# Daniel-Liu-c0deb0t/cute-nucleotides

Hardware: AMD Instinct MI355X
Metric: Gnt/s encode+decode on 16 GiB random ACGT; % HBM read roofline at 1/8 GPU (higher is better)
Workload: dtype u8

## Files before the change

### hip/counted_output.hpp

```cpp
#pragma once

#include <hip/hip_runtime.h>
#include <stdint.h>

#include <algorithm>
#include <initializer_list>

#include "util_kernels.hpp"
#include "word_tile.hpp"

namespace cnt {

constexpr int kCountedScanBlock = 1024, kCountedGroup = 16;

__device__ __forceinline__ uint64_t counted_tile_base(const uint64_t* offs, const uint32_t* counts, uint64_t tile) {
    uint64_t b = offs[tile / kCountedGroup];
    const uint32_t* g = counts + (tile - tile % kCountedGroup);
#pragma unroll
    for (int q = 0; q < kCountedGroup - 1; ++q) b += (uint64_t)q < tile % kCountedGroup ? g[q] : 0u;
    return b;
}

__global__ __launch_bounds__(kCountedScanBlock) void counted_scan(const uint32_t* __restrict__ counts, uint64_t* __restrict__ offs,
                                                                  uint64_t n_tiles, uint64_t* __restrict__ count) {
    __shared__ uint64_t s_w[kCountedScanBlock / 64];
    const uint32_t lane = threadIdx.x & 63, wave = threadIdx.x >> 6;
    const uint64_t n_groups = (n_tiles + kCountedGroup - 1) / kCountedGroup;
    uint64_t carry = 0;
    for (uint64_t first = 0; first < n_groups; first += kCountedScanBlock) {
        const uint64_t g = first + threadIdx.x;
        uint64_t sum = 0;
        if (g < n_groups) {
            const u32x4* q = reinterpret_cast<const u32x4*>(counts + g * kCountedGroup);
#pragma unroll
            for (int u = 0; u < kCountedGroup / 4; ++u) {
                const u32x4 c = q[u];
#pragma unroll
                for (int e = 0; e < 4; ++e) sum += g * kCountedGroup + 4 * u + e < n_tiles ? c[e] : 0u;
            }
        }
        uint64_t x = sum;
#pragma unroll
        for (int o = 1; o < 64; o <<= 1) {
            const uint64_t y = shfl_up_u64(x, o);
            if (lane >= (uint32_t)o) x += y;
        }
        if (lane == 63) s_w[wave] = x;
        __syncthreads();
        uint64_t before = carry + x - sum, total = 0;
#pragma unroll
        for (int q = 0; q < kCountedScanBlock / 64; ++q) {
            const uint64_t y = s_w[q];
            before += q < (int)wave ? y : 0;
            total += y;
        }
        if (g < n_groups) offs[g] = before;
        carry += total;
        __syncthreads();
    }
    if (threadIdx.x == 0) *count = carry;
}

inline uint64_t counted_scratch_bytes(uint64_t n_tiles) {
    if (!n_tiles) return 0;
    const uint64_t groups = (n_tiles + kCountedGroup - 1) / kCountedGroup;
    return 16 + ((groups + 1) & ~1ull) * 8 + groups * kCountedGroup * 4;
}

struct CountedScratch {
    uint64_t* offs;
    uint32_t* counts;
    void* behind;
};
inline CountedScratch counted_carve(void* d_work, uint64_t n_tiles) {
    const uint64_t groups = (n_tiles + kCountedGroup - 1) / kCountedGroup;
    uint64_t* offs = reinterpret_cast<uint64_t*>((reinterpret_cast<uintptr_t>(d_work) + 15) & ~(uintptr_t)15);
    uint32_t* counts = reinterpret_cast<uint32_t*>(offs + ((groups + 1) & ~1ull));
    return {offs, counts, counts + groups * kCountedGroup};
}

inline void counted_scan_enqueue(const CountedScratch& w, uint64_t n_tiles, void* d_count, hipStream_t s) {
    hipLaunchKernelGGL(counted_scan, dim3(1), dim3(kCountedScanBlock), 0, s, w.counts, w.offs, n_tiles, static_cast<uint64_t*>(d_count));
}

struct CountedOut {
    const void* p;
    bool required;
};
inline int counted_args(const void* bits, size_t len, std::initializer_list<CountedOut> outs, uint64_t most, size_t out_cap, const void* count) {
    if (!bits || !count || !aligned(bits, 8) || !aligned(count, 8)) return CNT_EINVAL;
    for (const CountedOut& o : outs)
        if ((o.required && !o.p) || !aligned(o.p, 8)) return CNT_EINVAL;
    const size_t in_bytes = cnt_words_for(len) * 8, out_bytes = std::min<uint64_t>(most, out_cap) * 8;
    if (overlaps(count, 8, bits, in_bytes)) return CNT_EINVAL;
    for (const CountedOut* o = outs.begin(); o != outs.end(); ++o) {
        if (!o->p) continue;
        if (overlaps(bits, in_bytes, o->p, out_bytes) || overlaps(count, 8, o->p, out_bytes)) return CNT_EINVAL;
        for (const CountedOut* e = outs.begin(); e != o; ++e)
            if (e->p && overlaps(e->p, out_bytes, o->p, out_bytes)) return CNT_EINVAL;
    }
    return CNT_OK;
}

inline int counted_work(const void* d_work, size_t work_bytes, size_t need, const void* bits, size_t len, std::initializer_list<const void*> outs,
                        uint64_t most, size_t out_cap, const void* count) {
    if (work_bytes < need || !d_work) return CNT_EINVAL;
    if (overlaps(d_work, need, bits, cnt_words_for(len) * 8) || overlaps(d_work, need, count, 8)) return CNT_EINVAL;
    for (const void* o : outs)
        if (o && overlaps(d_work, need, o, std::min<uint64_t>(most, out_cap) * 8)) return CNT_EINVAL;
    return CNT_OK;
}
// ... 23 lines not shown
```

### hip/orf_kernels.hpp

```cpp
#pragma once

#include <hip/hip_runtime.h>
#include <stdint.h>

#include "codec2_kernels.hpp"
#include "counted_output.hpp"
#include "find_kernels.hpp"

namespace cnt {

constexpr int kOrfBlock = 256;
constexpr int kOrfWaves = kOrfBlock / 64;
constexpr uint64_t kOrfTileWords = kOrfBlock, kOrfTile = 32 * kOrfTileWords;
constexpr int kOrfCarryBlock = 1024;
constexpr int kOrfPairs = 6;
constexpr uint32_t kOrfOpenEnd = 0x400u, kOrfNoStop = 0x800u;
constexpr uint64_t kOrfNone = ~0ull;
static_assert(kOrfTile + 1 < (1u << 16), "a position of a tile, plus one, is half a dword");

struct OrfArgs {
    const uint8_t* in;
    uint64_t words, len;
    uint64_t stops[2], starts[2];
    uint64_t min_len;
    uint64_t n_tiles;
    uint32_t* sums;
    uint64_t* carry;
    uint32_t* counts;
    uint64_t* offs;
    uint64_t *pos, *length, *info;
    uint64_t out_cap;
};

__device__ __forceinline__ uint32_t orf_combine(uint32_t a, uint32_t b, bool rev) {
    const uint32_t sa = a & 0xFFFFu, sb = b & 0xFFFFu;
    const uint32_t st = rev ? (sb ? sb : sa) : (sa ? sa : sb);
    return (b >> 16) ? b : ((a & 0xFFFF0000u) | st);
}

struct OrfLane {
    uint64_t i0;
    uint32_t stops[2], starts[2];
    uint32_t m3;
};

__device__ __forceinline__ OrfLane orf_lane(const OrfArgs& a, uint64_t tile, uint32_t* s_tab) {
    const uint32_t j = threadIdx.x;
    if (j < 64) {
        s_tab[j] = (uint32_t)((a.stops[0] >> j) & 1u) | ((uint32_t)((a.starts[0] >> j) & 1u) << 8) | ((uint32_t)((a.stops[1] >> j) & 1u) << 16) |
                   ((uint32_t)((a.starts[1] >> j) & 1u) << 24);
    }
    const uint64_t w0 = tile * kOrfTileWords;
    uint64_t lo, hi;
    word_tile_pair<kOrfTileWords>(a.in, a.words, w0, j, lo, hi);
    __syncthreads();
    const uint32_t d[3] = {(uint32_t)lo, (uint32_t)(lo >> 32), (uint32_t)hi};
    uint32_t acc[4];
#pragma unroll
    for (int g = 0; g < 4; ++g) {
        acc[g] = 0;
#pragma unroll
        for (int r = 8 * g + 7; r >= 8 * g; --r)
            acc[g] = (acc[g] << 1) | s_tab[window_dword(d, r) & 63u];
    }
    OrfLane L;
    L.i0 = (w0 + j) * 32;
    L.m3 = (2u * (uint32_t)(tile % 3) + 2u * j) % 3u;
// ... 14 lines not shown
    const uint32_t rel = threadIdx.x * 32u + 1u, lane = threadIdx.x & 63u;
#pragma unroll
    for (int p = 0; p < kOrfPairs; ++p) {
        const int s = p / 3;
        const uint32_t mask = 0x49249249u << ((p % 3 + 3u - L.m3) % 3u);
        const uint32_t st = L.stops[s] & mask;
        const uint32_t top = st ? 31u - (uint32_t)__builtin_clz(st) : 0u;
        const uint32_t sa = L.starts[s] & mask & (st ? ~((2u << top) - 1u) : ~0u);
        const uint32_t at = s ? 31u - (uint32_t)__builtin_clz(sa | 1u) : (uint32_t)__builtin_ctz(sa | 0x80000000u);
        x[p] = (st ? (rel + top) << 16 : 0u) | (sa ? rel + at : 0u);
    }
#pragma unroll
    for (int o = 1; o < 64; o <<= 1) {
#pragma unroll
        for (int p = 0; p < kOrfPairs; ++p) {
            if (p >= 3 && !both) continue;
            const uint32_t y = __shfl_up(x[p], o, 64);
            if (lane >= (uint32_t)o) x[p] = orf_combine(y, x[p], p >= 3);
        }
    }
}

__global__ __launch_bounds__(kOrfBlock) void orf_summary(OrfArgs a, uint64_t first_tile) {
    __shared__ uint32_t s_tab[64];
    __shared__ uint32_t s_w[kOrfWaves][kOrfPairs];
    const uint64_t tile = first_tile + blockIdx.x;
    const bool both = a.stops[1] != 0;
    const OrfLane L = orf_lane(a, tile, s_tab);
    uint32_t x[kOrfPairs];
    orf_wave_scan(L, both, x);
    if ((threadIdx.x & 63u) == 63u) {
#pragma unroll
        for (int p = 0; p < kOrfPairs; ++p) s_w[threadIdx.x >> 6][p] = x[p];
    }
    __syncthreads();
    if (threadIdx.x < (both ? kOrfPairs : 3)) {
        const uint32_t p = threadIdx.x;
        uint32_t v = 0;
#pragma unroll
        for (int q = 0; q < kOrfWaves; ++q) v = orf_combine(v, s_w[q][p], p >= 3);
        a.sums[p * a.n_tiles + tile] = v;
    }
}

__device__ __forceinline__ void orf_combine64(uint64_t& stop, uint64_t& start, uint64_t b_stop, uint64_t b_start, bool rev) {
    if (b_stop != kOrfNone) {
        stop = b_stop;
        start = b_start;
    } else if (rev ? b_start != kOrfNone : start == kOrfNone) {
        start = b_start;
    }
}

__global__ __launch_bounds__(kOrfCarryBlock) void orf_carry(const uint32_t* __restrict__ sums, uint64_t* __restrict__ carry, uint64_t n_tiles) {
    __shared__ uint64_t s_w[kOrfCarryBlock / 64][2];
    const uint32_t p = blockIdx.x, lane = threadIdx.x & 63u, wave = threadIdx.x >> 6;
    const bool rev = p >= 3;
    const uint32_t* in = sums + p * n_tiles;
    uint64_t* out_stop = carry + 2ull * p * n_tiles;
    uint64_t* out_start = out_stop + n_tiles;
    uint64_t c_stop = kOrfNone, c_start = kOrfNone;
    for (uint64_t first = 0; first < n_tiles; first += kOrfCarryBlock) {
        const uint64_t t = first + threadIdx.x;
        const uint32_t v = t < n_tiles ? in[t] : 0u;
        const uint64_t own_stop = (v >> 16) ? t * kOrfTile + (v >> 16) - 1 : kOrfNone, own_start = (v & 0xFFFFu) ? t * kOrfTile + (v & 0xFFFFu) - 1 : kOrfNone;
        uint64_t stop = own_stop, start = own_start;
#pragma unroll
        for (int o = 1; o < 64; o <<= 1) {
            uint64_t y_stop = shfl_up_u64(stop, o), y_start = shfl_up_u64(start, o);
            if (lane >= (uint32_t)o) {
                orf_combine64(y_stop, y_start, stop, start, rev);
                stop = y_stop;
                start = y_start;
            }
        }
        if (lane == 63) {
            s_w[wave][0] = stop;
            s_w[wave][1] = start;
        }
        uint64_t e_stop = shfl_up_u64(stop, 1), e_start = shfl_up_u64(start, 1);
        if (lane == 0) e_stop = e_start = kOrfNone;
        __syncthreads();
        uint64_t b_stop = c_stop, b_start = c_start;
#pragma unroll
        for (int q = 0; q < kOrfCarryBlock / 64; ++q) {
            if (q == (int)wave) {
                uint64_t f_stop = b_stop, f_start = b_start;
                orf_combine64(f_stop, f_start, e_stop, e_start, rev);
                if (t < n_tiles) {
                    out_stop[t] = f_stop;
                    out_start[t] = f_start;
                }
            }
            orf_combine64(b_stop, b_start, s_w[q][0], s_w[q][1], rev);
        }
        c_stop = b_stop;
        c_start = b_start;
        __syncthreads();
    }
}

template <bool WRITE>
__device__ __forceinline__ void orf_tile(const OrfArgs& a, uint64_t first_tile) {
    __shared__ uint32_t s_tab[64];
    __shared__ uint32_t s_w[kOrfWaves][kOrfPairs];
    __shared__ uint64_t s_carry[kOrfPairs][2];
    __shared__ uint32_t s_cnt[kOrfWaves];
    __shared__ uint64_t s_base;
    const uint64_t tile = first_tile + blockIdx.x;
    const uint32_t j = threadIdx.x, lane = j & 63u, wave = j >> 6;
    const bool both = a.stops[1] != 0, have_starts = (a.starts[0] | a.starts[1]) != 0;
    if constexpr (WRITE) {
        if (a.counts[tile] == 0) return;
    }
    if (j < 2 * kOrfPairs) s_carry[j >> 1][j & 1] = (both || j < 6) ? a.carry[j * a.n_tiles + tile] : kOrfNone;
    const OrfLane L = orf_lane(a, tile, s_tab);
    uint32_t x[kOrfPairs];
    orf_wave_scan(L, both, x);
    if (lane == 63) {
#pragma unroll
        for (int p = 0; p < kOrfPairs; ++p) s_w[wave][p] = x[p];
    }
    __syncthreads();
    uint32_t before[kOrfPairs];
#pragma unroll
    for (int p = 0; p < kOrfPairs; ++p) {
        uint32_t e = __shfl_up(x[p], 1, 64), v = 0;
        if (lane == 0) e = 0;
#pragma unroll
        for (int q = 0; q < kOrfWaves - 1; ++q) v = q < (int)wave ? orf_combine(v, s_w[q][p], p >= 3) : v;
        before[p] = orf_combine(v, e, p >= 3);
    }
    const uint64_t tile0 = tile * kOrfTile, m = a.len - 2;
    const uint32_t len3 = (uint32_t)(a.len % 3);

    uint64_t e_pos, e_len, e_info;
    auto entry = [&](int s, uint32_t r) -> bool {
        const uint32_t k = r % 3u, q = (L.m3 + k) % 3u;
        const uint32_t mask = (0x49249249u << k) & ((1u << r) - 1u);
        const uint32_t st = L.stops[s] & mask;
        const uint64_t hi = L.i0 + r;
        uint64_t lo, at;
        bool lo_end = false;
        if (st) {
            const uint32_t top = 31u - (uint32_t)__builtin_clz(st);
            const uint32_t sa = L.starts[s] & mask & ~((2u << top) - 1u);
            lo = L.i0 + top;
            at = !sa ? kOrfNone : L.i0 + (s ? 31u - (uint32_t)__builtin_clz(sa) : (uint32_t)__builtin_ctz(sa));
        } else {
            const uint32_t sa = L.starts[s] & mask;
            const uint32_t b = q == 0 ? before[3 * s] : q == 1 ? before[3 * s + 1] : before[3 * s + 2];
            uint64_t stop = s_carry[3 * s + q][0], start = s_carry[3 * s + q][1];
// ... 58 lines not shown
```

### hip/word_tile.hpp

```cpp
#pragma once

#include <hip/hip_runtime.h>
#include <stdint.h>

#include "codec2_kernels.hpp"

namespace cnt {

__device__ __forceinline__ void u64_pair(vu4 q, uint64_t& lo, uint64_t& hi) {
    lo = ((uint64_t)q[1] << 32) | q[0];
    hi = ((uint64_t)q[3] << 32) | q[2];
}
__device__ __forceinline__ vu4 pack_u64x2(uint64_t o0, uint64_t o1) {
    return vu4{(uint32_t)o0, (uint32_t)(o0 >> 32), (uint32_t)o1, (uint32_t)(o1 >> 32)};
}

template <uint64_t TILE_WORDS, uint64_t BACK = 0>
__device__ __forceinline__ void word_tile_pair(const uint8_t* __restrict__ in, uint64_t words, uint64_t w0, uint32_t j, uint64_t& lo, uint64_t& hi) {
    if (w0 >= BACK && w0 - BACK + TILE_WORDS + 1 <= words) {
        const __amdgpu_buffer_rsrc_t rin = rsrc_of(in + (w0 - BACK) * 8, (uint32_t)(TILE_WORDS + 1) * 8);
        u64_pair(__builtin_amdgcn_raw_buffer_load_b128(rin, j * 8, 0, kNT), lo, hi);
    } else {
        const uint64_t* in64 = reinterpret_cast<const uint64_t*>(in);
        const uint64_t w = w0 + j - BACK;
// ... 5 lines not shown
__device__ __forceinline__ uint64_t funnel64(uint64_t lo, uint64_t hi, uint32_t sh) { return (lo >> sh) | ((hi << 1) << (63 - sh)); }

__device__ __forceinline__ uint32_t window_dword(const uint32_t* d, uint32_t r) {
    const uint32_t i = r >> 4, sh = 2 * (r & 15u);
    return sh ? __builtin_amdgcn_alignbit(d[i + 1], d[i], sh) : d[i];
}

__device__ __forceinline__ uint32_t codes_below(uint64_t i0, uint64_t x) {
    return x <= i0 ? 0u : (x - i0 >= 32 ? ~0u : (1u << (uint32_t)(x - i0)) - 1u);
}

__device__ __forceinline__ uint32_t wave_inclusive_sum(uint32_t c, uint32_t lane) {
    uint32_t x = c;
#pragma unroll
    for (int o = 1; o < 64; o <<= 1) {
        const uint32_t y = __shfl_up(x, o, 64);
        if (lane >= (uint32_t)o) x += y;
    }
    return x;
}

__device__ __forceinline__ uint32_t tile_rank_post(uint32_t c, uint32_t* s_cnt) {
    const uint32_t x = wave_inclusive_sum(c, threadIdx.x & 63u);
    if ((threadIdx.x & 63u) == 63u) s_cnt[threadIdx.x >> 6] = x;
    return x;
}
template <int WAVES>
__device__ __forceinline__ uint32_t tile_total(const uint32_t* s_cnt) {
    uint32_t total = 0;
#pragma unroll
    for (int q = 0; q < WAVES; ++q) total += s_cnt[q];
    return total;
}
template <int WAVES>
__device__ __forceinline__ uint32_t tile_before(const uint32_t* s_cnt, uint32_t excl) {
#pragma unroll
    for (int q = 0; q < WAVES - 1; ++q) excl += q < (int)(threadIdx.x >> 6) ? s_cnt[q] : 0u;
    return excl;
}

__device__ __forceinline__ uint64_t reverse_codes64(uint64_t x) {
    x = __builtin_bitreverse64(x);
    return ((x >> 1) & 0x5555555555555555ull) | ((x & 0x5555555555555555ull) << 1);
}
__device__ __forceinline__ uint32_t reverse_codes32(uint32_t x) {
    x = __builtin_bitreverse32(x);
    return ((x >> 1) & 0x55555555u) | ((x & 0x55555555u) << 1);
}

__device__ __forceinline__ uint64_t shfl_up_u64(uint64_t v, int o) {
    const uint32_t lo = __shfl_up((uint32_t)v, o, 64), hi = __shfl_up((uint32_t)(v >> 32), o, 64);
    return ((uint64_t)hi << 32) | lo;
}
__device__ __forceinline__ uint64_t wave_sum_u64(uint64_t v) {
#pragma unroll
    for (int off = 32; off > 0; off >>= 1) {
        const uint32_t lo = __shfl_down((uint32_t)v, off, 64), hi = __shfl_down((uint32_t)(v >> 32), off, 64);
        v += ((uint64_t)hi << 32) | lo;
    }
    return v;
}

}
```

### hip/cute_nt.hip

```cpp
#include "../include/cute_nt.h"

#include <hip/hip_runtime.h>

#include <algorithm>
#include <atomic>
#include <chrono>
#include <condition_variable>
#include <cstdint>
#include <cstdio>
#include <cstdlib>
#include <cstring>
#include <functional>
#include <map>
#include <mutex>
#include <thread>
#include <vector>

#include <pthread.h>
#include <sched.h>
#include <sys/mman.h>
#include <sys/syscall.h>
#include <unistd.h>

#include "codec2_kernels.hpp"
// ... 4 lines not shown

using namespace cnt;

namespace {

inline int hip_rc(hipError_t e) {
    if (e == hipSuccess) return CNT_OK;
    (void)hipGetLastError();
    return -(int)e;
}

#define CNT_TRY(expr)                      \
    do {                                   \
        int _rc = (expr);                  \
        if (_rc != CNT_OK) return _rc;     \
    } while (0)
#define HIP_TRY(expr) CNT_TRY(hip_rc(expr))

inline bool aligned(const void* p, size_t a) { return (reinterpret_cast<uintptr_t>(p) & (a - 1)) == 0; }
inline bool overlaps(const void* a, size_t a_bytes, const void* b, size_t b_bytes) {
    const uintptr_t x = reinterpret_cast<uintptr_t>(a), y = reinterpret_cast<uintptr_t>(b);
    return a_bytes && b_bytes && x < y + b_bytes && y < x + a_bytes;
}

#ifdef CNT_LAB_VARIANTS
std::atomic<int> g_encode_variant{0};
std::atomic<int> g_decode_variant{0};
std::atomic<int> g_encode2_variant{0};
std::atomic<int> g_decode2_variant{0};
std::atomic<int> g_small_nt{1 << 17};
std::atomic<int> g_reduce_xi{1};
std::atomic<int> g_reduce_persistent{1};
std::atomic<int> g_hamming_order{0};
std::atomic<int> g_reduce_fallbacks{0};
std::atomic<int> g_round_trip_shape{0};
std::atomic<int> g_round_trip_cap{(int)kRoundTripDefaultCap};
inline int tune_encode() { return g_encode_variant.load(std::memory_order_relaxed); }
inline int tune_decode() { return g_decode_variant.load(std::memory_order_relaxed); }
inline int tune_encode2() { return g_encode2_variant.load(std::memory_order_relaxed); }
inline int tune_decode2() { return g_decode2_variant.load(std::memory_order_relaxed); }
inline size_t tune_small_nt() { return (size_t)g_small_nt.load(std::memory_order_relaxed); }
inline int tune_round_trip_shape() { return g_round_trip_shape.load(std::memory_order_relaxed); }
inline uint32_t tune_round_trip_cap() { return (uint32_t)g_round_trip_cap.load(std::memory_order_relaxed); }
std::atomic<int> g_round_trip_window_map{0};
inline int tune_round_trip_window_map() { return g_round_trip_window_map.load(std::memory_order_relaxed); }
std::atomic<int> g_round_trip_plan{kRoundTripDefaultPlan};
inline int tune_round_trip_plan() { return g_round_trip_plan.load(std::memory_order_relaxed); }
std::atomic<int> g_decode_rot{-1};
inline int tune_decode_rot() { return g_decode_rot.load(std::memory_order_relaxed); }
std::atomic<int> g_decode_window{1};
inline bool tune_decode_window() { return g_decode_window.load(std::memory_order_relaxed) != 0; }
std::atomic<int> g_kmer_count_lds_max_k{7};
inline int tune_kmer_count_lds_max_k() { return g_kmer_count_lds_max_k.load(std::memory_order_relaxed); }
std::atomic<int> g_decode_cache_log2{-1};
inline uint64_t decode_cache_nt() {
    const int o = g_decode_cache_log2.load(std::memory_order_relaxed);
    return o >= 0 ? (uint64_t)1 << o : chip_info().cache_nt;
}
#else
constexpr int tune_encode() { return 0; }
constexpr int tune_decode() { return 0; }
constexpr int tune_encode2() { return 0; }
constexpr int tune_decode2() { return 0; }
constexpr size_t tune_small_nt() { return (size_t)1 << 17; }
constexpr int tune_round_trip_shape() { return 0; }
constexpr uint32_t tune_round_trip_cap() { return kRoundTripDefaultCap; }
constexpr int tune_round_trip_window_map() { return 0; }
constexpr int tune_round_trip_plan() { return kRoundTripDefaultPlan; }
constexpr int tune_decode_rot() { return -1; }
constexpr bool tune_decode_window() { return true; }
constexpr int tune_kmer_count_lds_max_k() { return 7; }
inline uint64_t decode_cache_nt() { return chip_info().cache_nt; }
#endif

inline unsigned generic_grid(uint64_t items, unsigned block = kBlock) {
    return (unsigned)std::min<uint64_t>(std::max<uint64_t>((items + block - 1) / block, 1), 1u << 16);
}

template <typename F>
void split_launches(uint64_t n_tiles, int block, F&& launch) {
    for_each_launch(n_tiles, max_tiles_per_launch(block), [&](uint64_t first, uint64_t n, bool) { launch(first, n); });
}

int finish(hipStream_t s, int rc) {
    const int r2 = hip_rc(hipStreamSynchronize(s));
    return rc != CNT_OK ? rc : r2;
}

#include "shim_host_ctx.inc"
#include "device_tier.inc"
#include "host_tier.inc"
#include "sharded_tier.inc"

enum class Dir { in, out, counted };
struct HostBuf {
    const void* p;
    size_t bytes;
    Dir dir;
};

template <size_t N, typename F>
int host_call(const HostBuf (&b)[N], size_t aux_bytes, uint64_t* result, bool zero, F&& dev) {
    DevCtx* c = nullptr;
    CNT_TRY(t_ctx.get(&c));
    CNT_TRY(c->ensure_streams());
    void* d[N] = {};
    bool staged = false;
    for (size_t i = 0; i < N && !staged; ++i) {
        if (!b[i].p) continue;
        for (size_t j = 0; j < i; ++j)
            staged = staged || (b[j].p && (b[i].dir != Dir::in || b[j].dir != Dir::in) && overlaps(b[i].p, b[i].bytes, b[j].p, b[j].bytes));
        staged = staged || !host_range_is_pinned(b[i].p, b[i].bytes, &d[i]) || !d[i];
    }
    if (staged) {
        size_t at[N] = {}, tail = 0;
        for (size_t i = 1; i < N; ++i)
            if (b[i].p) {
                at[i] = tail;
                tail += (b[i].bytes + 7) & ~(size_t)7;
            }
        CNT_TRY(c->ensure_aux(0, b[0].bytes));
        if (N > 1) CNT_TRY(c->ensure_aux(1, std::max<size_t>(tail, 1)));
        for (size_t i = 0; i < N; ++i) d[i] = b[i].p ? static_cast<uint8_t*>(c->d_aux[i ? 1 : 0]) + at[i] : nullptr;
    }
// ... 416 lines not shown

int cnt_count_mismatch_dev(const void* d_a, const void* d_b, size_t nbytes, void* d_count, void* stream) {
    if (nbytes == 0) return CNT_OK;
    if (!d_a || !d_b || !d_count || !aligned(d_count, 8)) return CNT_EINVAL;
    hipLaunchKernelGGL(count_mismatch, dim3(std::min(generic_grid(nbytes >> 4), 4096u)), dim3(kBlock), 0,
                       static_cast<hipStream_t>(stream), static_cast<const uint8_t*>(d_a), static_cast<const uint8_t*>(d_b),
                       (uint64_t)nbytes, (aligned(d_a, 16) && aligned(d_b, 16)) ? 1 : 0,
                       static_cast<unsigned long long*>(d_count));
    return hip_rc(hipGetLastError());
}

int cnt_set_tuning(const char* key, int value) {
    if (!key) return CNT_EINVAL;
#ifdef CNT_LAB_VARIANTS
    if (!strcmp(key, "encode")) {
        if (value < 0 || value >= kNumEncodeVariants) return CNT_EINVAL;
        g_encode_variant.store(value);
    } else if (!strcmp(key, "decode")) {
        if (value < 0 || value >= kNumDecodeVariants) return CNT_EINVAL;
        g_decode_variant.store(value);
    } else if (!strcmp(key, "encode2")) {
        if (value < 0 || value >= kNumEncode2Variants) return CNT_EINVAL;
        g_encode2_variant.store(value);
    } else if (!strcmp(key, "decode2")) {
        if (value < 0 || value >= kNumDecode2Variants) return CNT_EINVAL;
        g_decode2_variant.store(value);
    } else if (!strcmp(key, "round_trip_cap")) {
        if (value < 0 || value > 32) return CNT_EINVAL;
        g_round_trip_cap.store(value);
    } else if (!strcmp(key, "round_trip_shape")) {
        if (value < 0 || value > 1) return CNT_EINVAL;
        g_round_trip_shape.store(value);
    } else if (!strcmp(key, "round_trip_window_map")) {
        if (value < 0 || value > 2) return CNT_EINVAL;
        g_round_trip_window_map.store(value);
    } else if (!strcmp(key, "round_trip_plan")) {
        if (value < 0 || value > 3) return CNT_EINVAL;
        g_round_trip_plan.store(value);
    } else if (!strcmp(key, "decode_window")) {
        if (value < 0 || value > 1) return CNT_EINVAL;
        g_decode_window.store(value);
    } else if (!strcmp(key, "decode_cache_log2")) {
        if (value < -1 || value > 40) return CNT_EINVAL;
        g_decode_cache_log2.store(value);
    } else if (!strcmp(key, "decode_rot")) {
        if (value < -1 || (value > 3 && value != 10 && value != 11)) return CNT_EINVAL;
        g_decode_rot.store(value);
    } else if (!strcmp(key, "reduce_persistent")) {
        if (value < 0 || value > 1) return CNT_EINVAL;
        g_reduce_persistent.store(value);
    } else if (!strcmp(key, "kmer_count_lds_max_k")) {
        if (value < 0 || value > 7) return CNT_EINVAL;
        g_kmer_count_lds_max_k.store(value);
    } else if (!strcmp(key, "hamming_order")) {
        if (value < 0 || value > 2) return CNT_EINVAL;
        g_hamming_order.store(value);
    } else if (!strcmp(key, "reduce_xi")) {
        if (value < 0 || value > 1) return CNT_EINVAL;
        g_reduce_xi.store(value);
    } else if (!strcmp(key, "xcd_shift")) {
        if (value < -1 || value > 6) return CNT_EINVAL;
        xcd_shift_override().store(value);
    } else if (!strcmp(key, "small_nt")) {
        if (value < 0) return CNT_EINVAL;
        g_small_nt.store(value);
    } else if (!strcmp(key, "launch_tiles")) {
        if (value < 0 || value % 64) return CNT_EINVAL;
        launch_tiles_override().store(value);
    } else {
        return CNT_EINVAL;
    }
    return CNT_OK;
#else
    (void)value;
    return CNT_EINVAL;
#endif
}

int cnt_get_tuning(const char* key, int* value) {
    if (!key || !value) return CNT_EINVAL;
    if (!strcmp(key, "lab_build")) {
#ifdef CNT_LAB_VARIANTS
        *value = 1;
#else
        *value = 0;
#endif
    } else if (!strcmp(key, "encode")) *value = tune_encode();
    else if (!strcmp(key, "decode")) *value = tune_decode();
    else if (!strcmp(key, "encode2")) *value = tune_encode2();
    else if (!strcmp(key, "decode2")) *value = tune_decode2();
    else if (!strcmp(key, "small_nt")) *value = (int)tune_small_nt();
    else if (!strcmp(key, "xcd_shift")) *value = (int)xcd_shift();
    else if (!strcmp(key, "round_trip_cap")) *value = (int)tune_round_trip_cap();
    else if (!strcmp(key, "round_trip_shape")) *value = tune_round_trip_shape();
    else if (!strcmp(key, "encode_variants")) *value = kNumEncodeVariants;
    else if (!strcmp(key, "decode_variants")) *value = kNumDecodeVariants;
    else if (!strcmp(key, "encode2_variants")) *value = kNumEncode2Variants;
    else if (!strcmp(key, "decode2_variants")) *value = kNumDecode2Variants;
    else if (!strcmp(key, "kmer_count_lds_max_k")) *value = tune_kmer_count_lds_max_k();
#ifdef CNT_LAB_VARIANTS
    else if (!strcmp(key, "launch_tiles")) *value = launch_tiles_override().load();
    else if (!strcmp(key, "decode_rot")) *value = g_decode_rot.load();
    else if (!strcmp(key, "decode_window")) *value = g_decode_window.load();
    else if (!strcmp(key, "decode_cache_log2")) *value = g_decode_cache_log2.load();
    else if (!strcmp(key, "reduce_xi")) *value = g_reduce_xi.load();
    else if (!strcmp(key, "hamming_order")) *value = g_hamming_order.load();
    else if (!strcmp(key, "reduce_fallbacks")) *value = g_reduce_fallbacks.load();
    else if (!strcmp(key, "reduce_persistent")) *value = g_reduce_persistent.load();
#else
    else if (!strcmp(key, "launch_tiles")) *value = 0;
    else if (!strcmp(key, "reduce_persistent")) *value = 1;
    else if (!strcmp(key, "reduce_fallbacks")) *value = 0;
#endif
    else return CNT_EINVAL;
    return CNT_OK;
}

int cnt_chip_info(int device, int* compute_units, int* lds_bytes_per_cu, int* xcds) {
    int count = 0;
    if (hipGetDeviceCount(&count) != hipSuccess || device < 0 || device >= count) return CNT_ENODEV;
    const ChipInfo c = query_chip(device);
    if (compute_units) *compute_units = (int)c.cus;
    if (lds_bytes_per_cu) *lds_bytes_per_cu = (int)c.lds_per_cu;
    if (xcds) *xcds = (int)c.xcds;
    return CNT_OK;
}

int cnt_chip_cache_nt(int device, uint64_t* nt) {
    int count = 0;
    if (!nt) return CNT_EINVAL;
    if (hipGetDeviceCount(&count) != hipSuccess || device < 0 || device >= count) return CNT_ENODEV;
    *nt = query_chip(device).cache_nt;
    return CNT_OK;
}

int cnt_check_device_range(const void* p, size_t bytes, int device) {
    if (!p) return CNT_EINVAL;
    int count = 0, cur = 0;
    if (hipGetDeviceCount(&count) != hipSuccess || count <= 0) return CNT_ENODEV;
    if (device < 0) {
        HIP_TRY(hipGetDevice(&cur));
        device = cur;
    }
    if (device >= count) return CNT_ENODEV;
    hipPointerAttribute_t a;
    if (hipPointerGetAttributes(&a, p) != hipSuccess) {
        (void)hipGetLastError();
        return CNT_EINVAL;
    }
    if (a.type == hipMemoryTypeDevice && a.device != device) {
        int peer = 0;
        if (hipDeviceCanAccessPeer(&peer, device, a.device) != hipSuccess || !peer) {
// ... 93 lines not shown
```

### hip/kmer_count_abi.inc

```
#include "kmer_count_kernels.hpp"

namespace {

int kmer_count_args(const void* bits, size_t len, unsigned k, unsigned flags, const void* counts, size_t counts_cap, bool host) {
    if (k == 0 || k > CNT_KMER_COUNTS_MAX_K || (flags & ~CNT_KMER_CANONICAL)) return CNT_EINVAL;
    if (len < k && !host) return CNT_OK;
    const uint64_t bins = (uint64_t)1 << (2 * k);
    if (!counts || !aligned(counts, 8)) return CNT_EINVAL;
    if (len >= k && (!bits || !aligned(bits, 8))) return CNT_EINVAL;
    if (counts_cap < bins) return CNT_ECAP;
    if (len >= k && overlaps(bits, cnt_words_for(len) * 8, counts, bins * 8)) return CNT_EINVAL;
    return CNT_OK;
}

static_assert(CNT_KMER_COUNTS_MAX_K == kKmerCountMaxK, "the header's constant is the kernels'");
#ifndef CNT_LAB_VARIANTS
static_assert(tune_kmer_count_lds_max_k() == kKmerCountLdsMaxK, "the product build counts in LDS up to kKmerCountLdsMaxK");
#endif

}

extern "C" {

int cnt_kmer_counts_dev(const void* d_bits, size_t len, unsigned k, unsigned flags, void* d_counts, size_t counts_cap, void* stream) {
    CNT_TRY(kmer_count_args(d_bits, len, k, flags, d_counts, counts_cap, false));
    if (len < k) return CNT_OK;
    hipStream_t s = static_cast<hipStream_t>(stream);
    const uint32_t canonical = (flags & CNT_KMER_CANONICAL) ? 1u : 0u;
    const uint64_t m = (uint64_t)len - k + 1, words = cnt_words_for(len);
    const uint64_t n_tiles = (m + kKmerCountTileKmers - 1) / kKmerCountTileKmers;
    const uint8_t* in8 = static_cast<const uint8_t*>(d_bits);
    unsigned long long* counts = static_cast<unsigned long long*>(d_counts);
    const uint64_t bound = (n_tiles + kKmerCountMaxTilesPerGroup - 1) / kKmerCountMaxTilesPerGroup;
    if ((int)k <= tune_kmer_count_lds_max_k()) {
        const unsigned grid = (unsigned)std::max<uint64_t>(std::min<uint64_t>(n_tiles, (uint64_t)chip_info().cus * 2), bound);
        hipLaunchKernelGGL((kmer_count<true>), dim3(grid), dim3(kKmerCountBlock), 0, s, in8, words, m, (uint32_t)k, canonical, n_tiles, counts);
    } else {
        const unsigned grid = (unsigned)std::min<uint64_t>(n_tiles, (uint64_t)chip_info().cus * 2);
        hipLaunchKernelGGL((kmer_count<false>), dim3(grid), dim3(kKmerCountBlock), 0, s, in8, words, m, (uint32_t)k, canonical, n_tiles, counts);
    }
    return hip_rc(hipGetLastError());
}

int cnt_kmer_counts(const uint64_t* bits, size_t len, unsigned k, unsigned flags, uint64_t* counts, size_t counts_cap) {
    CNT_TRY(kmer_count_args(bits, len, k, flags, counts, counts_cap, true));
    const size_t bytes = (size_t)8 << (2 * k);
    if (len < k) {
        memset(counts, 0, bytes);
        return CNT_OK;
    }
    std::vector<uint8_t> bounce;
    if (host_range_leaves_pinned(counts, bytes)) bounce.resize(bytes);
    void* dst = bounce.empty() ? static_cast<void*>(counts) : bounce.data();
    const HostBuf in[1] = {{bits, cnt_words_for(len) * 8, Dir::in}};
    CNT_TRY(host_call(in, bytes, nullptr, false, [&](void* const* d, void* aux, hipStream_t s) {
        HIP_TRY(hipMemsetAsync(aux, 0, bytes, s));
        CNT_TRY(cnt_kmer_counts_dev(d[0], len, k, flags, aux, bytes / 8, s));
        return hip_rc(hipMemcpyAsync(dst, aux, bytes, hipMemcpyDeviceToHost, s));
    }));
    if (!bounce.empty()) memcpy(counts, bounce.data(), bytes);
    return CNT_OK;
}

}
```

### hip/kmer_count_kernels.hpp

```cpp
#pragma once

#include <hip/hip_runtime.h>
#include <stdint.h>

#include "codec2_kernels.hpp"
#include "word_tile.hpp"

namespace cnt {

constexpr int kKmerCountMaxK = 12;
constexpr int kKmerCountLdsMaxK = 7;
constexpr int kKmerCountBlock = 1024;
constexpr uint32_t kKmerCountSlots = 16384;
constexpr uint32_t kKmerCountMaxReplicas = 256;
constexpr uint64_t kKmerCountTileWords = kKmerCountBlock, kKmerCountTileKmers = 32 * kKmerCountTileWords;
constexpr uint64_t kKmerCountMaxTilesPerGroup = (1ull << 17) - 1;
static_assert(kKmerCountMaxTilesPerGroup * kKmerCountTileKmers < (1ull << 32), "an LDS counter would wrap before its flush");
static_assert((1u << (2 * kKmerCountLdsMaxK)) <= kKmerCountSlots && kKmerCountSlots * 4 <= 65536, "the LDS table is at most 64 KiB");

__host__ __device__ constexpr uint32_t kmer_count_replica_log2(uint32_t k) {
    uint32_t r = 0;
    while ((2u << r) <= kKmerCountMaxReplicas && ((uint64_t)(2u << r) << (2 * k)) <= kKmerCountSlots) ++r;
    return r;
}

template <bool CANONICAL>
__device__ __forceinline__ uint32_t kmer_count_finish(uint32_t fwd, uint32_t k) {
    if constexpr (CANONICAL) {
        const uint32_t rc = reverse_codes32(fwd ^ 0xAAAAAAAAu) >> (32 - 2 * k);
        return rc < fwd ? rc : fwd;
    } else {
        return fwd;
    }
}

template <bool LDS>
__device__ __forceinline__ void kmer_count_add(uint32_t* table, unsigned long long* counts, uint32_t v, uint32_t run, uint32_t rlog, uint32_t rep) {
    if constexpr (LDS) atomicAdd(&table[(v << rlog) + rep], run);
    else atomicAdd(&counts[v], (unsigned long long)run);
}

template <bool LDS, bool CANONICAL, bool FULL>
__device__ __forceinline__ void kmer_count_lane(uint64_t lo, uint64_t hi, uint32_t nv, uint32_t k, uint32_t mask, uint32_t* table,
                                                unsigned long long* counts, uint32_t rlog, uint32_t rep) {
    uint32_t prev = 0, run = 0;
#pragma unroll
    for (uint32_t r = 0; r < 32; ++r) {
        if (FULL || r < nv) {
            const uint32_t win = r == 0 ? (uint32_t)lo : (uint32_t)((lo >> (2 * r)) | (hi << (64 - 2 * r)));
            const uint32_t v = kmer_count_finish<CANONICAL>(win & mask, k);
            if (run != 0 && v != prev) {
                kmer_count_add<LDS>(table, counts, prev, run, rlog, rep);
                run = 0;
            }
            prev = v;
            ++run;
        }
    }
    if (run != 0) kmer_count_add<LDS>(table, counts, prev, run, rlog, rep);
}

template <bool LDS>
__global__ __launch_bounds__(kKmerCountBlock) void kmer_count(const uint8_t* __restrict__ in, uint64_t words, uint64_t m, uint32_t k, uint32_t canonical,
                                                             uint64_t n_tiles, unsigned long long* __restrict__ counts) {
    __shared__ uint32_t table[LDS ? kKmerCountSlots : 1];
    const uint32_t j = threadIdx.x, rlog = kmer_count_replica_log2(k), rep = j & ((1u << rlog) - 1u);
    const uint32_t mask = (1u << (2 * k)) - 1u;
    if constexpr (LDS) {
        for (uint32_t i = j; i < kKmerCountSlots; i += kKmerCountBlock) table[i] = 0;
        __syncthreads();
    }
    auto load = [&](uint64_t t, uint64_t& lo, uint64_t& hi) { word_tile_pair<kKmerCountTileWords>(in, words, t * kKmerCountTileWords, j, lo, hi); };
    uint64_t t = blockIdx.x, lo = 0, hi = 0;
    if (t < n_tiles) load(t, lo, hi);
    while (t < n_tiles) {
        const uint64_t tn = t + gridDim.x, cur_lo = lo, cur_hi = hi;
        if (tn < n_tiles) load(tn, lo, hi);
        const uint64_t i0 = (t * kKmerCountTileWords + j) * 32;
        if ((t + 1) * kKmerCountTileKmers <= m) {
            if (canonical) kmer_count_lane<LDS, true, true>(cur_lo, cur_hi, 32, k, mask, table, counts, rlog, rep);
            else kmer_count_lane<LDS, false, true>(cur_lo, cur_hi, 32, k, mask, table, counts, rlog, rep);
        } else {
            const uint32_t nv = i0 >= m ? 0u : (uint32_t)(m - i0 < 32 ? m - i0 : 32);
            if (canonical) kmer_count_lane<LDS, true, false>(cur_lo, cur_hi, nv, k, mask, table, counts, rlog, rep);
            else kmer_count_lane<LDS, false, false>(cur_lo, cur_hi, nv, k, mask, table, counts, rlog, rep);
        }
        t = tn;
    }
    if constexpr (LDS) {
        __syncthreads();
        const uint32_t bins = 1u << (2 * k), reps = 1u << rlog;
        for (uint32_t b0 = j; b0 < bins; b0 += kKmerCountBlock) {
            const uint32_t b = (b0 + blockIdx.x * 64u) & (bins - 1u);
            uint64_t sum = 0;
            for (uint32_t r = 0; r < reps; ++r) sum += table[(b << rlog) + ((r + j) & (reps - 1u))];
            if (sum) atomicAdd(&counts[b], (unsigned long long)sum);
        }
    }
}

}
```

Baseline: 5545.

## Prefetch next round in single-block scans and batch ORF carry per thread

The single-block counted_scan and orf_carry kernels now load the next round's inputs one iteration ahead, using double-buffered shared memory so the trailing __syncthreads can be dropped. orf_carry also handles four tiles per thread, does the in-round scan with 32-bit relative positions, and replaces the serial loop over waves with a wave-level shuffle scan. This aims to cut latency in these serial, one-block scan kernels that sit between the main passes. In exchange the code is more complex and uses a hand-written s_waitcnt immediate and a sched_barrier, which depend on the target's encoding.

```diff
diff --git a/hip/counted_output.hpp b/hip/counted_output.hpp
--- a/hip/counted_output.hpp
+++ b/hip/counted_output.hpp
@@ -23,40 +23,55 @@
 
 __global__ __launch_bounds__(kCountedScanBlock) void counted_scan(const uint32_t* __restrict__ counts, uint64_t* __restrict__ offs,
                                                                   uint64_t n_tiles, uint64_t* __restrict__ count) {
-    __shared__ uint64_t s_w[kCountedScanBlock / 64];
+    __shared__ uint64_t s_w[2][kCountedScanBlock / 64];
     const uint32_t lane = threadIdx.x & 63, wave = threadIdx.x >> 6;
     const uint64_t n_groups = (n_tiles + kCountedGroup - 1) / kCountedGroup;
+    if (n_groups == 0) {
+        if (threadIdx.x == 0) *count = 0;
+        return;
+    }
+    auto load = [&](uint64_t g, u32x4(&c)[kCountedGroup / 4]) {
+        const u32x4* q = reinterpret_cast<const u32x4*>(counts + (g < n_groups ? g : 0) * kCountedGroup);
+#pragma unroll
+        for (int u = 0; u < kCountedGroup / 4; ++u) c[u] = q[u];
+    };
+    auto group_sum = [&](uint64_t g, const u32x4(&c)[kCountedGroup / 4]) {
+        uint64_t sum = 0;
+#pragma unroll
+        for (int u = 0; u < kCountedGroup / 4; ++u) {
+#pragma unroll
+            for (int e = 0; e < 4; ++e) sum += g * kCountedGroup + 4 * u + e < n_tiles ? c[u][e] : 0u;
+        }
+        return sum;
+    };
     uint64_t carry = 0;
-    for (uint64_t first = 0; first < n_groups; first += kCountedScanBlock) {
+    u32x4 ahead[kCountedGroup / 4];
+    load(threadIdx.x, ahead);
+    uint64_t sum = group_sum(threadIdx.x, ahead);
+    load(kCountedScanBlock + threadIdx.x, ahead);
+    uint32_t buf = 0;
+    for (uint64_t first = 0; first < n_groups; first += kCountedScanBlock, buf ^= 1u) {
         const uint64_t g = first + threadIdx.x;
-        uint64_t sum = 0;
-        if (g < n_groups) {
-            const u32x4* q = reinterpret_cast<const u32x4*>(counts + g * kCountedGroup);
-#pragma unroll
-            for (int u = 0; u < kCountedGroup / 4; ++u) {
-                const u32x4 c = q[u];
-#pragma unroll
-                for (int e = 0; e < 4; ++e) sum += g * kCountedGroup + 4 * u + e < n_tiles ? c[e] : 0u;
-            }
-        }
         uint64_t x = sum;
 #pragma unroll
         for (int o = 1; o < 64; o <<= 1) {
             const uint64_t y = shfl_up_u64(x, o);
             if (lane >= (uint32_t)o) x += y;
         }
-        if (lane == 63) s_w[wave] = x;
+        if (lane == 63) s_w[buf][wave] = x;
         __syncthreads();
         uint64_t before = carry + x - sum, total = 0;
 #pragma unroll
         for (int q = 0; q < kCountedScanBlock / 64; ++q) {
-            const uint64_t y = s_w[q];
+            const uint64_t y = s_w[buf][q];
             before += q < (int)wave ? y : 0;
             total += y;
         }
+        carry += total;
+        wait_vector_memory();
         if (g < n_groups) offs[g] = before;
-        carry += total;
-        __syncthreads();
+        sum = group_sum(g + kCountedScanBlock, ahead);
+        load(g + 2 * kCountedScanBlock, ahead);
     }
     if (threadIdx.x == 0) *count = carry;
 }
diff --git a/hip/orf_kernels.hpp b/hip/orf_kernels.hpp
--- a/hip/orf_kernels.hpp
+++ b/hip/orf_kernels.hpp
@@ -12,7 +12,8 @@
 constexpr int kOrfBlock = 256;
 constexpr int kOrfWaves = kOrfBlock / 64;
 constexpr uint64_t kOrfTileWords = kOrfBlock, kOrfTile = 32 * kOrfTileWords;
-constexpr int kOrfCarryBlock = 1024;
+constexpr int kOrfCarryBlock = 1024, kOrfCarryTiles = 4;
+constexpr uint64_t kOrfCarryRound = (uint64_t)kOrfCarryBlock * kOrfCarryTiles;
 constexpr int kOrfPairs = 6;
 constexpr uint32_t kOrfOpenEnd = 0x400u, kOrfNoStop = 0x800u;
 constexpr uint64_t kOrfNone = ~0ull;
@@ -133,52 +134,104 @@
     }
 }
 
-__global__ __launch_bounds__(kOrfCarryBlock) void orf_carry(const uint32_t* __restrict__ sums, uint64_t* __restrict__ carry, uint64_t n_tiles) {
-    __shared__ uint64_t s_w[kOrfCarryBlock / 64][2];
+static_assert(kOrfCarryRound * kOrfTile < (1ull << 32), "a position of a round, plus one, is a dword");
+__device__ __forceinline__ void orf_combine_round(uint32_t& stop, uint32_t& start, uint32_t b_stop, uint32_t b_start, bool rev) {
+    const bool take = b_stop || (rev ? b_start != 0 : start == 0);
+    stop = b_stop ? b_stop : stop;
+    start = take ? b_start : start;
+}
+__device__ __forceinline__ uint32_t orf_round_stop(uint32_t local, uint32_t v) { return (v >> 16) ? local * (uint32_t)kOrfTile + (v >> 16) : 0u; }
+__device__ __forceinline__ uint32_t orf_round_start(uint32_t local, uint32_t v) { return (v & 0xFFFFu) ? local * (uint32_t)kOrfTile + (v & 0xFFFFu) : 0u; }
+
+__device__ __forceinline__ void orf_carry_load(const uint32_t* __restrict__ in, uint64_t n_tiles, uint64_t t0, uint32_t (&v)[kOrfCarryTiles]) {
+    const uint32_t* q = in + (t0 < n_tiles ? t0 : 0);
+#pragma unroll
+    for (int k = 0; k < kOrfCarryTiles; ++k) v[k] = q[k];
+}
+__device__ __forceinline__ void orf_carry_mask(uint64_t n_tiles, uint64_t t0, const uint32_t (&raw)[kOrfCarryTiles], uint32_t (&v)[kOrfCarryTiles]) {
+#pragma unroll
+    for (int k = 0; k < kOrfCarryTiles; ++k) v[k] = t0 + k < n_tiles ? raw[k] : 0u;
+}
+
+template <bool REV>
+__device__ __forceinline__ void orf_carry_pair(const uint32_t* __restrict__ sums, uint64_t* __restrict__ carry, uint64_t n_tiles,
+                                               uint32_t (&s_w)[2][kOrfCarryBlock / 64][2]) {
+    constexpr uint32_t kWaves = kOrfCarryBlock / 64;
+    static_assert(kWaves <= 64 && (kWaves & (kWaves - 1)) == 0, "a wave scans the waves' values in aligned groups of lanes");
     const uint32_t p = blockIdx.x, lane = threadIdx.x & 63u, wave = threadIdx.x >> 6;
-    const bool rev = p >= 3;
     const uint32_t* in = sums + p * n_tiles;
     uint64_t* out_stop = carry + 2ull * p * n_tiles;
     uint64_t* out_start = out_stop + n_tiles;
+    const uint32_t own = threadIdx.x * kOrfCarryTiles;
     uint64_t c_stop = kOrfNone, c_start = kOrfNone;
-    for (uint64_t first = 0; first < n_tiles; first += kOrfCarryBlock) {
-        const uint64_t t = first + threadIdx.x;
-        const uint32_t v = t < n_tiles ? in[t] : 0u;
-        const uint64_t own_stop = (v >> 16) ? t * kOrfTile + (v >> 16) - 1 : kOrfNone, own_start = (v & 0xFFFFu) ? t * kOrfTile + (v & 0xFFFFu) - 1 : kOrfNone;
-        uint64_t stop = own_stop, start = own_start;
+    uint32_t v[kOrfCarryTiles], ahead[kOrfCarryTiles];
+    orf_carry_load(in, n_tiles, own, ahead);
+    orf_carry_mask(n_tiles, own, ahead, v);
+    orf_carry_load(in, n_tiles, own + kOrfCarryRound, ahead);
+    uint32_t buf = 0;
+    for (uint64_t first = 0; first < n_tiles; first += kOrfCarryRound, buf ^= 1u) {
+        uint32_t stop = 0, start = 0;
+#pragma unroll
+        for (int k = 0; k < kOrfCarryTiles; ++k) orf_combine_round(stop, start, orf_round_stop(own + k, v[k]), orf_round_start(own + k, v[k]), REV);
 #pragma unroll
         for (int o = 1; o < 64; o <<= 1) {
-            uint64_t y_stop = shfl_up_u64(stop, o), y_start = shfl_up_u64(start, o);
+            uint32_t y_stop = __shfl_up(stop, o, 64), y_start = __shfl_up(start, o, 64);
             if (lane >= (uint32_t)o) {
-                orf_combine64(y_stop, y_start, stop, start, rev);
+                orf_combine_round(y_stop, y_start, stop, start, REV);
                 stop = y_stop;
                 start = y_start;
             }
         }
         if (lane == 63) {
-            s_w[wave][0] = stop;
-            s_w[wave][1] = start;
-        }
-        uint64_t e_stop = shfl_up_u64(stop, 1), e_start = shfl_up_u64(start, 1);
-        if (lane == 0) e_stop = e_start = kOrfNone;
+            s_w[buf][wave][0] = stop;
+            s_w[buf][wave][1] = start;
+        }
+        uint32_t r_stop = __shfl_up(stop, 1, 64), r_start = __shfl_up(start, 1, 64);
+        if (lane == 0) r_stop = r_start = 0;
         __syncthreads();
-        uint64_t b_stop = c_stop, b_start = c_start;
-#pragma unroll
-        for (int q = 0; q < kOrfCarryBlock / 64; ++q) {
-            if (q == (int)wave) {
-                uint64_t f_stop = b_stop, f_start = b_start;
-                orf_combine64(f_stop, f_start, e_stop, e_start, rev);
-                if (t < n_tiles) {
-                    out_stop[t] = f_stop;
-                    out_start[t] = f_start;
-                }
+        const uint32_t sub = lane % kWaves;
+        uint32_t w_stop = s_w[buf][sub][0], w_start = s_w[buf][sub][1];
+#pragma unroll
+        for (int o = 1; o < (int)kWaves; o <<= 1) {
+            uint32_t y_stop = __shfl_up(w_stop, o, 64), y_start = __shfl_up(w_start, o, 64);
+            if (sub >= (uint32_t)o) {
+                orf_combine_round(y_stop, y_start, w_stop, w_start, REV);
+                w_stop = y_stop;
+                w_start = y_start;
             }
-            orf_combine64(b_stop, b_start, s_w[q][0], s_w[q][1], rev);
-        }
-        c_stop = b_stop;
-        c_start = b_start;
-        __syncthreads();
-    }
+        }
+        uint32_t q_stop = __shfl(w_stop, (wave + kWaves - 1) % kWaves, 64), q_start = __shfl(w_start, (wave + kWaves - 1) % kWaves, 64);
+        if (wave == 0) q_stop = q_start = 0;
+        orf_combine_round(q_stop, q_start, r_stop, r_start, REV);
+        r_stop = q_stop;
+        r_start = q_start;
+        const uint32_t all_stop = __shfl(w_stop, kWaves - 1, 64), all_start = __shfl(w_start, kWaves - 1, 64);
+        const uint64_t base = first * kOrfTile - 1;
+        wait_vector_memory();
+#pragma unroll
+        for (int k = 0; k < kOrfCarryTiles; ++k) {
+            const uint64_t t = first + own + k;
+            uint64_t f_stop = c_stop, f_start = c_start;
+            orf_combine64(f_stop, f_start, r_stop ? base + r_stop : kOrfNone, r_start ? base + r_start : kOrfNone, REV);
+            if (t < n_tiles) {
+                out_stop[t] = f_stop;
+                out_start[t] = f_start;
+            }
+            orf_combine_round(r_stop, r_start, orf_round_stop(own + k, v[k]), orf_round_start(own + k, v[k]), REV);
+        }
+        orf_combine64(c_stop, c_start, all_stop ? base + all_stop : kOrfNone, all_start ? base + all_start : kOrfNone, REV);
+        orf_carry_mask(n_tiles, first + kOrfCarryRound + own, ahead, v);
+        orf_carry_load(in, n_tiles, first + 2 * kOrfCarryRound + own, ahead);
+    }
+}
+
+__global__ __launch_bounds__(kOrfCarryBlock) void orf_carry(const uint32_t* __restrict__ sums, uint64_t* __restrict__ carry, uint64_t n_tiles) {
+    __shared__ uint32_t s_w[2][kOrfCarryBlock / 64][2];
+    if (n_tiles == 0) return;
+    if (blockIdx.x >= 3)
+        orf_carry_pair<true>(sums, carry, n_tiles, s_w);
+    else
+        orf_carry_pair<false>(sums, carry, n_tiles, s_w);
 }
 
 template <bool WRITE>
diff --git a/hip/word_tile.hpp b/hip/word_tile.hpp
--- a/hip/word_tile.hpp
+++ b/hip/word_tile.hpp
@@ -81,6 +81,10 @@
     const uint32_t lo = __shfl_up((uint32_t)v, o, 64), hi = __shfl_up((uint32_t)(v >> 32), o, 64);
     return ((uint64_t)hi << 32) | lo;
 }
+__device__ __forceinline__ uint64_t shfl_u64(uint64_t v, int src) {
+    const uint32_t lo = __shfl((uint32_t)v, src, 64), hi = __shfl((uint32_t)(v >> 32), src, 64);
+    return ((uint64_t)hi << 32) | lo;
+}
 __device__ __forceinline__ uint64_t wave_sum_u64(uint64_t v) {
 #pragma unroll
     for (int off = 32; off > 0; off >>= 1) {
@@ -90,4 +94,9 @@
     return v;
 }
 
+__device__ __forceinline__ void wait_vector_memory() {
+    __builtin_amdgcn_sched_barrier(0);
+    __builtin_amdgcn_s_waitcnt(0x0F70);
 }
+
+}
```

After: 5541. About the same (-0.1%).

## Count mid-size k-mers in LDS bin slices instead of global atomics

Applied to the files above, without the earlier changes.

For k between the LDS-table limit and a new slice limit (default 10), the k-mer bin space is split into fixed 32K-entry slices, one per grid row. Each workgroup counts only the k-mers that fall in its slice into shared memory, then flushes the non-zero bins to global counters. This replaces per-run 64-bit global atomics with LDS atomics. In exchange, every slice row re-reads the whole input, and a tuning knob with a matching static_assert is added.

```diff
diff --git a/hip/cute_nt.hip b/hip/cute_nt.hip
--- a/hip/cute_nt.hip
+++ b/hip/cute_nt.hip
@@ -80,6 +80,8 @@
 inline bool tune_decode_window() { return g_decode_window.load(std::memory_order_relaxed) != 0; }
 std::atomic<int> g_kmer_count_lds_max_k{7};
 inline int tune_kmer_count_lds_max_k() { return g_kmer_count_lds_max_k.load(std::memory_order_relaxed); }
+std::atomic<int> g_kmer_count_slice_max_k{10};
+inline int tune_kmer_count_slice_max_k() { return g_kmer_count_slice_max_k.load(std::memory_order_relaxed); }
 std::atomic<int> g_decode_cache_log2{-1};
 inline uint64_t decode_cache_nt() {
     const int o = g_decode_cache_log2.load(std::memory_order_relaxed);
@@ -98,6 +100,7 @@
 constexpr int tune_decode_rot() { return -1; }
 constexpr bool tune_decode_window() { return true; }
 constexpr int tune_kmer_count_lds_max_k() { return 7; }
+constexpr int tune_kmer_count_slice_max_k() { return 10; }
 inline uint64_t decode_cache_nt() { return chip_info().cache_nt; }
 #endif
 
@@ -620,6 +623,9 @@
     } else if (!strcmp(key, "kmer_count_lds_max_k")) {
         if (value < 0 || value > 7) return CNT_EINVAL;
         g_kmer_count_lds_max_k.store(value);
+    } else if (!strcmp(key, "kmer_count_slice_max_k")) {
+        if (value < 7 || value > 12) return CNT_EINVAL;
+        g_kmer_count_slice_max_k.store(value);
     } else if (!strcmp(key, "hamming_order")) {
         if (value < 0 || value > 2) return CNT_EINVAL;
         g_hamming_order.store(value);
@@ -666,6 +672,7 @@
     else if (!strcmp(key, "encode2_variants")) *value = kNumEncode2Variants;
     else if (!strcmp(key, "decode2_variants")) *value = kNumDecode2Variants;
     else if (!strcmp(key, "kmer_count_lds_max_k")) *value = tune_kmer_count_lds_max_k();
+    else if (!strcmp(key, "kmer_count_slice_max_k")) *value = tune_kmer_count_slice_max_k();
 #ifdef CNT_LAB_VARIANTS
     else if (!strcmp(key, "launch_tiles")) *value = launch_tiles_override().load();
     else if (!strcmp(key, "decode_rot")) *value = g_decode_rot.load();
diff --git a/hip/kmer_count_abi.inc b/hip/kmer_count_abi.inc
--- a/hip/kmer_count_abi.inc
+++ b/hip/kmer_count_abi.inc
@@ -16,6 +16,7 @@
 static_assert(CNT_KMER_COUNTS_MAX_K == kKmerCountMaxK, "the header's constant is the kernels'");
 #ifndef CNT_LAB_VARIANTS
 static_assert(tune_kmer_count_lds_max_k() == kKmerCountLdsMaxK, "the product build counts in LDS up to kKmerCountLdsMaxK");
+static_assert(tune_kmer_count_slice_max_k() == kKmerCountSliceMaxK, "the product build counts in LDS bin slices up to kKmerCountSliceMaxK");
 #endif
 
 }
@@ -35,6 +36,11 @@
     if ((int)k <= tune_kmer_count_lds_max_k()) {
         const unsigned grid = (unsigned)std::max<uint64_t>(std::min<uint64_t>(n_tiles, (uint64_t)chip_info().cus * 2), bound);
         hipLaunchKernelGGL((kmer_count<true>), dim3(grid), dim3(kKmerCountBlock), 0, s, in8, words, m, (uint32_t)k, canonical, n_tiles, counts);
+    } else if ((int)k > kKmerCountLdsMaxK && (int)k <= tune_kmer_count_slice_max_k()) {
+        const uint64_t slices = ((uint64_t)1 << (2 * k)) / kKmerCountSliceSlots, resident = (uint64_t)chip_info().cus * kKmerCountSliceGroupsPerCu;
+        const uint64_t per_slice = std::max<uint64_t>({1, (resident + slices - 1) / slices, bound});
+        const dim3 grid((unsigned)std::min<uint64_t>(per_slice, n_tiles), (unsigned)slices);
+        hipLaunchKernelGGL(kmer_count_sliced, grid, dim3(kKmerCountBlock), 0, s, in8, words, m, (uint32_t)k, canonical, n_tiles, counts);
     } else {
         const unsigned grid = (unsigned)std::min<uint64_t>(n_tiles, (uint64_t)chip_info().cus * 2);
         hipLaunchKernelGGL((kmer_count<false>), dim3(grid), dim3(kKmerCountBlock), 0, s, in8, words, m, (uint32_t)k, canonical, n_tiles, counts);
diff --git a/hip/kmer_count_kernels.hpp b/hip/kmer_count_kernels.hpp
--- a/hip/kmer_count_kernels.hpp
+++ b/hip/kmer_count_kernels.hpp
@@ -17,6 +17,14 @@
 constexpr uint64_t kKmerCountMaxTilesPerGroup = (1ull << 17) - 1;
 static_assert(kKmerCountMaxTilesPerGroup * kKmerCountTileKmers < (1ull << 32), "an LDS counter would wrap before its flush");
 static_assert((1u << (2 * kKmerCountLdsMaxK)) <= kKmerCountSlots && kKmerCountSlots * 4 <= 65536, "the LDS table is at most 64 KiB");
+constexpr int kKmerCountSliceMaxK = 10;
+constexpr uint32_t kKmerCountSliceSlots = 32768;
+constexpr uint32_t kKmerCountSliceGroupsPerCu = kKmerCountSliceSlots * 4 <= 65536 ? 2 : 1;
+static_assert(kKmerCountLdsMaxK <= kKmerCountSliceMaxK && kKmerCountSliceMaxK <= kKmerCountMaxK, "LDS table, then slices, then global adds");
+static_assert((kKmerCountSliceSlots & (kKmerCountSliceSlots - 1)) == 0 && kKmerCountSliceSlots % kKmerCountBlock == 0 && kKmerCountSliceSlots * 4 <= 131072 &&
+                  kKmerCountSliceSlots <= (1u << (2 * (kKmerCountLdsMaxK + 1))),
+              "S = 4^k / kKmerCountSliceSlots whole slices (S >= 1) cover the 4^k bins of every sliced k, a slice fits the LDS");
+enum : int { kKmerCountGlobal = 0, kKmerCountLds = 1, kKmerCountSliced = 2 };
 
 __host__ __device__ constexpr uint32_t kmer_count_replica_log2(uint32_t k) {
     uint32_t r = 0;
@@ -34,13 +42,15 @@
     }
 }
 
-template <bool LDS>
+template <int REGIME>
 __device__ __forceinline__ void kmer_count_add(uint32_t* table, unsigned long long* counts, uint32_t v, uint32_t run, uint32_t rlog, uint32_t rep) {
-    if constexpr (LDS) atomicAdd(&table[(v << rlog) + rep], run);
-    else atomicAdd(&counts[v], (unsigned long long)run);
+    if constexpr (REGIME == kKmerCountLds) atomicAdd(&table[(v << rlog) + rep], run);
+    else if constexpr (REGIME == kKmerCountSliced) {
+        if (v - rep < kKmerCountSliceSlots) atomicAdd(&table[v - rep], run);
+    } else atomicAdd(&counts[v], (unsigned long long)run);
 }
 
-template <bool LDS, bool CANONICAL, bool FULL>
+template <int REGIME, bool CANONICAL, bool FULL>
 __device__ __forceinline__ void kmer_count_lane(uint64_t lo, uint64_t hi, uint32_t nv, uint32_t k, uint32_t mask, uint32_t* table,
                                                 unsigned long long* counts, uint32_t rlog, uint32_t rep) {
     uint32_t prev = 0, run = 0;
@@ -50,14 +60,14 @@
             const uint32_t win = r == 0 ? (uint32_t)lo : (uint32_t)((lo >> (2 * r)) | (hi << (64 - 2 * r)));
             const uint32_t v = kmer_count_finish<CANONICAL>(win & mask, k);
             if (run != 0 && v != prev) {
-                kmer_count_add<LDS>(table, counts, prev, run, rlog, rep);
+                kmer_count_add<REGIME>(table, counts, prev, run, rlog, rep);
                 run = 0;
             }
             prev = v;
             ++run;
         }
     }
-    if (run != 0) kmer_count_add<LDS>(table, counts, prev, run, rlog, rep);
+    if (run != 0) kmer_count_add<REGIME>(table, counts, prev, run, rlog, rep);
 }
 
 template <bool LDS>
@@ -99,4 +109,36 @@
     }
 }
 
+__global__ __launch_bounds__(kKmerCountBlock) void kmer_count_sliced(const uint8_t* __restrict__ in, uint64_t words, uint64_t m, uint32_t k, uint32_t canonical,
+                                                                    uint64_t n_tiles, unsigned long long* __restrict__ counts) {
+    __shared__ uint32_t table[kKmerCountSliceSlots];
+    const uint32_t j = threadIdx.x, first = blockIdx.y * kKmerCountSliceSlots;
+    const uint32_t mask = (1u << (2 * k)) - 1u;
+    for (uint32_t i = j; i < kKmerCountSliceSlots; i += kKmerCountBlock) table[i] = 0;
+    __syncthreads();
+    auto load = [&](uint64_t t, uint64_t& lo, uint64_t& hi) { word_tile_pair<kKmerCountTileWords>(in, words, t * kKmerCountTileWords, j, lo, hi); };
+    uint64_t t = blockIdx.x, lo = 0, hi = 0;
+    if (t < n_tiles) load(t, lo, hi);
+    while (t < n_tiles) {
+        const uint64_t tn = t + gridDim.x, cur_lo = lo, cur_hi = hi;
+        if (tn < n_tiles) load(tn, lo, hi);
+        const uint64_t i0 = (t * kKmerCountTileWords + j) * 32;
+        if ((t + 1) * kKmerCountTileKmers <= m) {
+            if (canonical) kmer_count_lane<kKmerCountSliced, true, true>(cur_lo, cur_hi, 32, k, mask, table, counts, 0, first);
+            else kmer_count_lane<kKmerCountSliced, false, true>(cur_lo, cur_hi, 32, k, mask, table, counts, 0, first);
+        } else {
+            const uint32_t nv = i0 >= m ? 0u : (uint32_t)(m - i0 < 32 ? m - i0 : 32);
+            if (canonical) kmer_count_lane<kKmerCountSliced, true, false>(cur_lo, cur_hi, nv, k, mask, table, counts, 0, first);
+            else kmer_count_lane<kKmerCountSliced, false, false>(cur_lo, cur_hi, nv, k, mask, table, counts, 0, first);
+        }
+        t = tn;
+    }
+    __syncthreads();
+    for (uint32_t b0 = j; b0 < kKmerCountSliceSlots; b0 += kKmerCountBlock) {
+        const uint32_t b = (b0 + blockIdx.x * 64u) & (kKmerCountSliceSlots - 1u);
+        const uint32_t c = table[b];
+        if (c) atomicAdd(&counts[first + b], (unsigned long long)c);
+    }
 }
+
+}
```

Measured after the change: 5529 before, 5529 after (median of 2 runs). No clear change (-0.0%).
